# coolbeam/UPFlow_pytorch

Measured on AMD Instinct MI355X. Metric: frame-pairs/sec at 384x1280 bf16, higher is better.
Workload: dtype bf16; 1 GPU; config2: UPFlow_net inference forward (flow fwd+bwd, occlusion masks, SGU on), 384x1280, batch 4 per GPU, random-init weights; global_batch=4, parallelism=replicas x1 (image pairs sharded, no collective), ranks=1, hip_graph=True, capture_fallback=False, steps_in_flight=4, pyramid_convs=HIP (MFMA kernel), pyramid_dtype=fp16

## Files before the change

### upflow_pytorch_amd/csrc/conv_pair.hip

```cpp
#include "conv_kernel.hpp"

namespace upf {
namespace convp {

using conv::f32x16;
using conv::Mma32;
using conv::u32x2;

constexpr int NT = 256;
template <int SA, int SB, int TH> struct Geo {
  static constexpr int MR = SB * (TH - 1) + 3, MC = SB * 31 + 3;
  static constexpr int XO = (SA == 2) ? 1 : 0;
  static constexpr int IR = SA * (MR - 1) + 3, IC = (SA * (MC - 1) + 3 + XO + 1) / 2 * 2;
};

template <typename T, int K0, int C1O, int TH, bool YC8, int SA, int SB>
__global__ __launch_bounds__(NT, 2)
void conv_pair_kernel(const T* __restrict__ x, long long xbs, int xpitch, int Cin, const T* __restrict__ wa, const float* __restrict__ ba, float slope_a,
                      const T* __restrict__ wb, const float* __restrict__ bb, float slope_b, T* __restrict__ y, long long ybs, int ypitch, int C2,
                      int H, int W, int Hm, int Wm, int Ho, int Wo, int tiles_x, int tiles_y) {
  using G = Geo<SA, SB, TH>;
  constexpr int MR = G::MR, MC = G::MC, IR = G::IR, IC = G::IC, XO = G::XO;
  constexpr bool QUAD = (K0 == 0);
  constexpr int KO = QUAD ? 1 : K0;
  constexpr int NSTEP = QUAD ? 3 : ((K0 == 1) ? 5 : 9);
  constexpr int KSB = C1O / 2;
  constexpr int RPWB = TH / 4;
  extern __shared__ __attribute__((aligned(16))) uint4 lds[];
  uint4* in_s = lds;
  uint4* mid_s = lds + (QUAD ? (IR * IC + 1) / 2 : K0 * IR * IC);

  const int bid = xcd_remap(blockIdx.x, gridDim.x);
  const int tx = bid % tiles_x, ty = (bid / tiles_x) % tiles_y, n = bid / (tiles_x * tiles_y);
  const int x0 = tx * 32, y0 = ty * TH;
  const int my0 = SB * y0 - 1, mx0 = SB * x0 - 1;
  const int tid = threadIdx.x, lane = tid & 63, wave = tid >> 6;
  const int px = lane & 31, kg = lane >> 5;

  {
    const uint32_t plane = (uint32_t)(H * xpitch) * 2u;
    __amdgpu_buffer_rsrc_t xr = __builtin_amdgcn_make_buffer_rsrc(const_cast<T*>(x + (size_t)n * xbs), 0, (uint32_t)Cin * plane, 0x00020000);
    const int iy0 = SA * my0 - 1, ix0 = SA * mx0 - 1 - XO;
    for (int item = tid; item < IR * (IC / 2); item += NT) {
      const int ir = item / (IC / 2), pp = item - ir * (IC / 2);
      const int gy = iy0 + ir, gx = ix0 + 2 * pp;
      const bool in = gy >= 0 && gy < H && gx >= 0 && gx < W;
      const uint32_t off = in ? (uint32_t)(gy * xpitch + gx) * 2u : 0x80000000u;
      const uint32_t hm = (gx + 1 < W) ? 0xffffffffu : 0x0000ffffu;
      if constexpr (QUAD) {
        uint32_t ch[4];
#pragma unroll
        for (int c = 0; c < 4; ++c) ch[c] = __builtin_amdgcn_raw_buffer_load_b32(xr, off + (uint32_t)c * plane, 0, 0) & hm;
        uint2 e0, e1;
        e0.x = __builtin_amdgcn_perm(ch[1], ch[0], 0x05040100u); e1.x = __builtin_amdgcn_perm(ch[1], ch[0], 0x07060302u);
        e0.y = __builtin_amdgcn_perm(ch[3], ch[2], 0x05040100u); e1.y = __builtin_amdgcn_perm(ch[3], ch[2], 0x07060302u);
        uint2* q = reinterpret_cast<uint2*>(in_s);
        q[ir * IC + 2 * pp] = e0;
        q[ir * IC + 2 * pp + 1] = e1;
      }
#pragma unroll
      for (int o = 0; o < K0; ++o) {
        uint32_t ch[8];
#pragma unroll
        for (int c = 0; c < 8; ++c)
          ch[c] = __builtin_amdgcn_raw_buffer_load_b32(xr, off + (uint32_t)(8 * o + c) * plane, 0, 0) & hm;
        uint4 e0, e1;
        e0.x = __builtin_amdgcn_perm(ch[1], ch[0], 0x05040100u); e1.x = __builtin_amdgcn_perm(ch[1], ch[0], 0x07060302u);
        e0.y = __builtin_amdgcn_perm(ch[3], ch[2], 0x05040100u); e1.y = __builtin_amdgcn_perm(ch[3], ch[2], 0x07060302u);
        e0.z = __builtin_amdgcn_perm(ch[5], ch[4], 0x05040100u); e1.z = __builtin_amdgcn_perm(ch[5], ch[4], 0x07060302u);
        e0.w = __builtin_amdgcn_perm(ch[7], ch[6], 0x05040100u); e1.w = __builtin_amdgcn_perm(ch[7], ch[6], 0x07060302u);
        in_s[(o * IR + ir) * IC + 2 * pp] = e0;
        in_s[(o * IR + ir) * IC + 2 * pp + 1] = e1;
      }
    }
  }
  uint4 wA[NSTEP];
#pragma unroll
  for (int s = 0; s < NSTEP; ++s) wA[s] = *reinterpret_cast<const uint4*>(wa + ((size_t)s * 64 + lane) * 8);
  constexpr int C1 = 8 * C1O;
  f32x16 biasA;
#pragma unroll
  for (int e = 0; e < 16; ++e) {
    const int c = (e & 3) + 8 * (e >> 2) + 4 * kg;
    biasA[e] = (c < C1) ? ba[c] : 0.f;
  }
  int offA[NSTEP], offA2[NSTEP];
#pragma unroll
  for (int s = 0; s < NSTEP; ++s) {
    int tap, oct;
    if constexpr (QUAD) { tap = 4 * s + 2 * kg; oct = 0; }
    else if constexpr (K0 == 1) { tap = 2 * s + kg; oct = 0; }
    else { tap = s; oct = kg; }
    const int t1 = tap > 8 ? 8 : tap, t2 = tap + 1 > 8 ? 8 : tap + 1;
    offA[s] = (oct * IR + t1 / 3) * IC + t1 % 3 + XO;
    offA2[s] = (t2 / 3) * IC + t2 % 3 + XO;
  }
  __syncthreads();

  {
    constexpr int NPX = MR * MC, NTILE = (NPX + 31) / 32;
    for (int t = wave; t < NTILE; t += 4) {
      const int p = t * 32 + px;
      const bool pv = p < NPX;
      const int pc = pv ? p : NPX - 1;
      const int mr = pc / MC, mc = pc - mr * MC;
      f32x16 acc = biasA;
      if constexpr (QUAD) {
        const uint2* ib = reinterpret_cast<const uint2*>(in_s) + SA * (mr * IC + mc);
#pragma unroll
        for (int s = 0; s < NSTEP; ++s) {
          const uint2 lo = ib[offA[s]], hi = ib[offA2[s]];
          acc = Mma32<T>::mma(wA[s], make_uint4(lo.x, lo.y, hi.x, hi.y), acc);
        }
      } else {
        const uint4* ib = in_s + SA * (mr * IC + mc);
#pragma unroll
        for (int s = 0; s < NSTEP; ++s) acc = Mma32<T>::mma(wA[s], ib[offA[s]], acc);
      }
      const int my = my0 + mr, mx = mx0 + mc;
      const bool inside = my >= 0 && my < Hm && mx >= 0 && mx < Wm;
      if (pv) {
#pragma unroll
        for (int o = 0; o < C1O; ++o) {
          float v[4];
#pragma unroll
          for (int q = 0; q < 4; ++q) { v[q] = acc[4 * o + q]; v[q] = fmaxf(v[q], v[q] * slope_a); }
          u32x2 w2;
          w2.x = inside ? pack2<T>(v[0], v[1]) : 0u;
          w2.y = inside ? pack2<T>(v[2], v[3]) : 0u;
          *reinterpret_cast<u32x2*>(reinterpret_cast<unsigned char*>(&mid_s[(o * MR + mr) * MC + mc]) + kg * 8) = w2;
        }
      }
    }
  }
  uint4 wB[9][KSB];
#pragma unroll
  for (int tap = 0; tap < 9; ++tap)
#pragma unroll
    for (int ks = 0; ks < KSB; ++ks) wB[tap][ks] = *reinterpret_cast<const uint4*>(wb + ((size_t)(tap * KSB + ks) * 64 + lane) * 8);
  f32x16 acc[RPWB];
#pragma unroll
  for (int e = 0; e < 16; ++e) {
    const int c = (e & 3) + 8 * (e >> 2) + 4 * kg;
    const float bv = (c < C2) ? bb[c] : 0.f;
#pragma unroll
    for (int rr = 0; rr < RPWB; ++rr) acc[rr][e] = bv;
  }
  __syncthreads();

#pragma unroll
  for (int tap = 0; tap < 9; ++tap) {
    const int ky = tap / 3, kx = tap - 3 * ky;
#pragma unroll
    for (int ks = 0; ks < KSB; ++ks)
#pragma unroll
      for (int rr = 0; rr < RPWB; ++rr) {
        const int r = wave * RPWB + rr;
        const uint4 b = mid_s[((2 * ks + kg) * MR + SB * r + ky) * MC + SB * px + kx];
        acc[rr] = Mma32<T>::mma(wB[tap][ks], b, acc[rr]);
      }
  }
  if constexpr (!YC8) {
    if (((ypitch & 7) | (int)(ybs & 7) | (int)(reinterpret_cast<uintptr_t>(y) & 15)) == 0) {
      __syncthreads();
      conv::epilogue_wide<T, RPWB>(acc, reinterpret_cast<unsigned char*>(lds) + wave * conv::EPI_WAVE_BYTES, y + (size_t)n * ybs, C2, Ho, Wo,
                                   0, lane, x0, __builtin_amdgcn_readfirstlane(y0 + wave * RPWB), 1, slope_b, ypitch);
      return;
    }
  }
  const int gx = x0 + px;
#pragma unroll
  for (int rr = 0; rr < RPWB; ++rr) {
    const int gy = y0 + wave * RPWB + rr;
    if (gy >= Ho || gx >= Wo) continue;
    if constexpr (YC8) {
      T* yo = y + (size_t)n * ybs;
#pragma unroll
      for (int g = 0; g < 4; ++g) {
        if (8 * g >= C2) continue;
        float v[4];
#pragma unroll
        for (int q = 0; q < 4; ++q) { v[q] = acc[rr][4 * g + q]; v[q] = fmaxf(v[q], v[q] * slope_b); }
        u32x2 o2;
        o2.x = pack2<T>(v[0], v[1]); o2.y = pack2<T>(v[2], v[3]);
        *reinterpret_cast<u32x2*>(yo + (((size_t)g * Ho + gy) * Wo + gx) * 8 + kg * 4) = o2;
      }
    } else {
      typename Elem<T>::store_t* yo = reinterpret_cast<typename Elem<T>::store_t*>(y + (size_t)n * ybs);
#pragma unroll
      for (int e = 0; e < 16; e += 2) {
        const int c = (e & 3) + 8 * (e >> 2) + 4 * kg;
        float v0 = acc[rr][e], v1 = acc[rr][e + 1];
        v0 = fmaxf(v0, v0 * slope_b); v1 = fmaxf(v1, v1 * slope_b);
        const uint32_t p2 = pack2<T>(v0, v1);
        if (c < C2) yo[((size_t)c * Ho + gy) * ypitch + gx] = (typename Elem<T>::store_t)(p2 & 0xffffu);
        if (c + 1 < C2) yo[((size_t)(c + 1) * Ho + gy) * ypitch + gx] = (typename Elem<T>::store_t)(p2 >> 16);
      }
    }
  }
}

struct PairArgs {
  const void* x; long long xbs; int xpitch, Cin; const void* wa; const float* ba; float slope_a; int C1;
  const void* wb; const float* bb; float slope_b; int C2; void* y; long long ybs; int ypitch; int B, H, W; hipStream_t stream;
  int sa, sb;
};

template <typename T, int K0, int C1O, int TH, bool YC8, int SA, int SB>
int launch_pair(const PairArgs& a) {
  using G = Geo<SA, SB, TH>;
  const int Hm = (a.H - 1) / SA + 1, Wm = (a.W - 1) / SA + 1;
  const int Ho = (Hm - 1) / SB + 1, Wo = (Wm - 1) / SB + 1;
  const int tiles_x = cdiv(Wo, 32), tiles_y = cdiv(Ho, TH);
  const size_t ldsb = (size_t)((K0 == 0 ? (G::IR * G::IC + 1) / 2 : K0 * G::IR * G::IC) + C1O * G::MR * G::MC) * 16;
  static LdsOptIn opt;
  auto kern = &conv_pair_kernel<T, K0, C1O, TH, YC8, SA, SB>;
  opt.ensure(reinterpret_cast<const void*>(kern), ldsb);
  hipLaunchKernelGGL(kern, dim3((unsigned)(a.B * tiles_x * tiles_y)), dim3(NT), ldsb, a.stream, (const T*)a.x, a.xbs, a.xpitch, a.Cin,
                     (const T*)a.wa, a.ba, a.slope_a, (const T*)a.wb, a.bb, a.slope_b, (T*)a.y, a.ybs, a.ypitch, a.C2, a.H, a.W, Hm, Wm, Ho, Wo, tiles_x, tiles_y);
  return check_launch("conv_pair_forward");
}

template <typename T, bool YC8>
int dispatch_pair(const PairArgs& a) {
  const int k0 = a.Cin <= 4 ? 0 : (a.Cin <= 8 ? 1 : 2), c1o = a.C1 / 8;
  if (a.sa == 1) {
    if (k0 == 0 && c1o == 2) return launch_pair<T, 0, 2, 8, YC8, 1, 2>(a);
    if (k0 == 0 && c1o == 4) return launch_pair<T, 0, 4, 4, YC8, 1, 2>(a);
    if (k0 == 1 && c1o == 2 && conv::g_pair_th == 4) return launch_pair<T, 1, 2, 4, YC8, 1, 2>(a);
    if (k0 == 1 && c1o == 2) return launch_pair<T, 1, 2, 8, YC8, 1, 2>(a);
    if (k0 == 1 && c1o == 4) return launch_pair<T, 1, 4, 4, YC8, 1, 2>(a);
    if (k0 == 2 && c1o == 2) return launch_pair<T, 2, 2, 8, YC8, 1, 2>(a);
    return launch_pair<T, 2, 4, 4, YC8, 1, 2>(a);
  }
  if constexpr (!YC8) {
    if (k0 == 0 && c1o == 2) return launch_pair<T, 0, 2, 8, false, 2, 1>(a);
    if (k0 == 0 && c1o == 4) return launch_pair<T, 0, 4, 8, false, 2, 1>(a);
    if (k0 == 1 && c1o == 2 && conv::g_pair_th == 4) return launch_pair<T, 1, 2, 4, false, 2, 1>(a);
    if (k0 == 1 && c1o == 2) return launch_pair<T, 1, 2, 8, false, 2, 1>(a);
    if (k0 == 1 && c1o == 4) return launch_pair<T, 1, 4, 8, false, 2, 1>(a);
    if (k0 == 2 && c1o == 2) return launch_pair<T, 2, 2, 8, false, 2, 1>(a);
    return launch_pair<T, 2, 4, 8, false, 2, 1>(a);
  }
  set_error("conv_pair_forward: [stride 2, stride 1] writes NCHW");
  return UPF_EUNSUPPORTED;
}

}
}

extern "C" int upf_conv_pair_forward(const void* x, long long x_batch_stride, int x_row_pitch, int Cin,
                                     const void* wa_packed, const float* bias_a, float slope_a, int C1, int stride_a,
                                     const void* wb_packed, const float* bias_b, float slope_b, int C2, int stride_b,
                                     void* y, long long y_batch_stride, int y_row_pitch, int y_is_c8,
                                     int B, int H, int W, int dtype, void* stream) {
  using namespace upf;
  UPF_REQUIRE(x && wa_packed && bias_a && wb_packed && bias_b && y, UPF_EINVAL, "conv_pair_forward: null pointer");
  UPF_REQUIRE(B > 0 && H > 0 && W > 0, UPF_EINVAL, "conv_pair_forward: bad shape B=%d H=%d W=%d", B, H, W);
  UPF_REQUIRE(dtype == UPF_BF16 || dtype == UPF_F16, UPF_EDTYPE, "conv_pair_forward: bf16 / fp16 only");
  UPF_REQUIRE(Cin >= 1 && Cin <= 16 && (C1 == 16 || C1 == 32) && C2 >= 1 && C2 <= 32, UPF_EUNSUPPORTED,
              "conv_pair_forward: Cin <= 16, C1 = 16 | 32, C2 <= 32 (got %d, %d, %d)", Cin, C1, C2);
  UPF_REQUIRE((stride_a == 1 && stride_b == 2) || (stride_a == 2 && stride_b == 1), UPF_EUNSUPPORTED,
              "conv_pair_forward: strides (1, 2) or (2, 1), got (%d, %d)", stride_a, stride_b);
  if (x_row_pitch == 0) x_row_pitch = W;
  const int Ho = (H - 1) / 2 + 1, Wo = (W - 1) / 2 + 1;
  if (y_row_pitch == 0) y_row_pitch = Wo;
  UPF_REQUIRE(x_row_pitch >= W && x_row_pitch % 2 == 0 && aligned_to(x, 4) && x_batch_stride % 2 == 0, UPF_EUNSUPPORTED,
              "conv_pair_forward: the input rows are read as pixel pairs: an even row pitch (%d) and a 4-byte aligned base", x_row_pitch);
  UPF_REQUIRE(slope_a >= 0.f && slope_a <= 1.f && slope_b >= 0.f && slope_b <= 1.f, UPF_EINVAL, "conv_pair_forward: leaky slopes in [0,1]");
  UPF_REQUIRE(aligned_to(wa_packed, 16) && aligned_to(wb_packed, 16), UPF_EINVAL, "conv_pair_forward: packed weights must be 16-byte aligned");
  UPF_REQUIRE(y_is_c8 ? (aligned_to(y, 16) && y_batch_stride % 8 == 0) : (y_row_pitch >= Wo), UPF_EINVAL, "conv_pair_forward: bad output layout");
  UPF_REQUIRE((long long)Cin * H * x_row_pitch * 2 < (1ll << 31), UPF_EINVAL, "conv_pair_forward: image too large for one buffer descriptor");
  convp::PairArgs a{x, x_batch_stride, x_row_pitch, Cin, wa_packed, bias_a, slope_a == 0.f ? 1.f : slope_a, C1,
                    wb_packed, bias_b, slope_b == 0.f ? 1.f : slope_b, C2, y, y_batch_stride, y_row_pitch, B, H, W, (hipStream_t)stream, stride_a, stride_b};
  if (dtype == UPF_BF16) return y_is_c8 ? convp::dispatch_pair<bf16_t, true>(a) : convp::dispatch_pair<bf16_t, false>(a);
  return y_is_c8 ? convp::dispatch_pair<f16_t, true>(a) : convp::dispatch_pair<f16_t, false>(a);
}
```

Baseline: 1928 frame-pairs/s.

## Software-pipeline LDS loads and MFMAs in fused conv-pair kernel

Restructures the fused two-conv kernel so that global input loads are all issued before the permute/store phase, the first conv's LDS operand fetch is double/triple-buffered ahead of its MFMAs with sched barriers, and the second conv preloads the next kernel row of LDS operands while computing the current one. Adds a spare LDS slot so invalid-pixel stores go to a dummy location instead of branching, and raises the occupancy hint to 3 workgroups for the small quad-input variant when LDS allows. The goal is to hide LDS and global latency behind MFMA work. The cost is higher register pressure, which may cause spills or lower occupancy.

```diff
diff --git a/upflow_pytorch_amd/csrc/conv_pair.hip b/upflow_pytorch_amd/csrc/conv_pair.hip
--- a/upflow_pytorch_amd/csrc/conv_pair.hip
+++ b/upflow_pytorch_amd/csrc/conv_pair.hip
@@ -14,8 +14,16 @@
   static constexpr int IR = SA * (MR - 1) + 3, IC = (SA * (MC - 1) + 3 + XO + 1) / 2 * 2;
 };
 
+template <int K0, int C1O, int TH, int SA, int SB> constexpr int pair_lds_bytes() {
+  using G = Geo<SA, SB, TH>;
+  return ((K0 == 0 ? (G::IR * G::IC + 1) / 2 : K0 * G::IR * G::IC) + C1O * G::MR * G::MC + 1) * 16;
+}
+template <int K0, int C1O, int TH, int SA, int SB> constexpr int pair_min_wg() {
+  return (K0 == 0 && C1O == 2 && 160 * 1024 / pair_lds_bytes<K0, C1O, TH, SA, SB>() >= 3) ? 3 : 2;
+}
+
 template <typename T, int K0, int C1O, int TH, bool YC8, int SA, int SB>
-__global__ __launch_bounds__(NT, 2)
+__global__ __launch_bounds__(NT, (pair_min_wg<K0, C1O, TH, SA, SB>()))
 void conv_pair_kernel(const T* __restrict__ x, long long xbs, int xpitch, int Cin, const T* __restrict__ wa, const float* __restrict__ ba, float slope_a,
                       const T* __restrict__ wb, const float* __restrict__ bb, float slope_b, T* __restrict__ y, long long ybs, int ypitch, int C2,
                       int H, int W, int Hm, int Wm, int Ho, int Wo, int tiles_x, int tiles_y) {
@@ -38,39 +46,53 @@
   const int px = lane & 31, kg = lane >> 5;
 
   {
+    constexpr int NPAIR = IR * (IC / 2), NITEM = (NPAIR + NT - 1) / NT, NPL = QUAD ? 4 : 8 * K0;
     const uint32_t plane = (uint32_t)(H * xpitch) * 2u;
     __amdgpu_buffer_rsrc_t xr = __builtin_amdgcn_make_buffer_rsrc(const_cast<T*>(x + (size_t)n * xbs), 0, (uint32_t)Cin * plane, 0x00020000);
     const int iy0 = SA * my0 - 1, ix0 = SA * mx0 - 1 - XO;
-    for (int item = tid; item < IR * (IC / 2); item += NT) {
-      const int ir = item / (IC / 2), pp = item - ir * (IC / 2);
+    uint32_t ch[NITEM][NPL], hm[NITEM];
+    int dst[NITEM];
+    int ir = tid / (IC / 2), pp = tid - ir * (IC / 2);
+#pragma unroll
+    for (int i = 0; i < NITEM; ++i) {
+      if ((i + 1) * NT > NPAIR) {
+        const bool past = i * NT + tid >= NPAIR;
+        ir = past ? IR - 1 : ir; pp = past ? IC / 2 - 1 : pp;
+      }
       const int gy = iy0 + ir, gx = ix0 + 2 * pp;
-      const bool in = gy >= 0 && gy < H && gx >= 0 && gx < W;
+      const bool in = ((unsigned)gy < (unsigned)H) & ((unsigned)gx < (unsigned)W);
       const uint32_t off = in ? (uint32_t)(gy * xpitch + gx) * 2u : 0x80000000u;
-      const uint32_t hm = (gx + 1 < W) ? 0xffffffffu : 0x0000ffffu;
+      hm[i] = (gx + 1 < W) ? 0xffffffffu : 0x0000ffffu;
+      dst[i] = ir * IC + 2 * pp;
+#pragma unroll
+      for (int c = 0; c < NPL; ++c)
+        ch[i][c] = __builtin_amdgcn_raw_buffer_load_b32(xr, off + (uint32_t)c * plane, 0, 0);
+      ir += NT / (IC / 2); pp += NT % (IC / 2);
+      if (pp >= IC / 2) { pp -= IC / 2; ++ir; }
+    }
+#pragma unroll
+    for (int i = 0; i < NITEM; ++i) {
       if constexpr (QUAD) {
-        uint32_t ch[4];
-#pragma unroll
-        for (int c = 0; c < 4; ++c) ch[c] = __builtin_amdgcn_raw_buffer_load_b32(xr, off + (uint32_t)c * plane, 0, 0) & hm;
+        const uint32_t c0 = ch[i][0] & hm[i], c1 = ch[i][1] & hm[i], c2 = ch[i][2] & hm[i], c3 = ch[i][3] & hm[i];
         uint2 e0, e1;
-        e0.x = __builtin_amdgcn_perm(ch[1], ch[0], 0x05040100u); e1.x = __builtin_amdgcn_perm(ch[1], ch[0], 0x07060302u);
-        e0.y = __builtin_amdgcn_perm(ch[3], ch[2], 0x05040100u); e1.y = __builtin_amdgcn_perm(ch[3], ch[2], 0x07060302u);
+        e0.x = __builtin_amdgcn_perm(c1, c0, 0x05040100u); e1.x = __builtin_amdgcn_perm(c1, c0, 0x07060302u);
+        e0.y = __builtin_amdgcn_perm(c3, c2, 0x05040100u); e1.y = __builtin_amdgcn_perm(c3, c2, 0x07060302u);
         uint2* q = reinterpret_cast<uint2*>(in_s);
-        q[ir * IC + 2 * pp] = e0;
-        q[ir * IC + 2 * pp + 1] = e1;
+        q[dst[i]] = e0;
+        q[dst[i] + 1] = e1;
       }
 #pragma unroll
       for (int o = 0; o < K0; ++o) {
-        uint32_t ch[8];
-#pragma unroll
-        for (int c = 0; c < 8; ++c)
-          ch[c] = __builtin_amdgcn_raw_buffer_load_b32(xr, off + (uint32_t)(8 * o + c) * plane, 0, 0) & hm;
+        uint32_t c[8];
+#pragma unroll
+        for (int j = 0; j < 8; ++j) c[j] = ch[i][8 * o + j] & hm[i];
         uint4 e0, e1;
-        e0.x = __builtin_amdgcn_perm(ch[1], ch[0], 0x05040100u); e1.x = __builtin_amdgcn_perm(ch[1], ch[0], 0x07060302u);
-        e0.y = __builtin_amdgcn_perm(ch[3], ch[2], 0x05040100u); e1.y = __builtin_amdgcn_perm(ch[3], ch[2], 0x07060302u);
-        e0.z = __builtin_amdgcn_perm(ch[5], ch[4], 0x05040100u); e1.z = __builtin_amdgcn_perm(ch[5], ch[4], 0x07060302u);
-        e0.w = __builtin_amdgcn_perm(ch[7], ch[6], 0x05040100u); e1.w = __builtin_amdgcn_perm(ch[7], ch[6], 0x07060302u);
-        in_s[(o * IR + ir) * IC + 2 * pp] = e0;
-        in_s[(o * IR + ir) * IC + 2 * pp + 1] = e1;
+        e0.x = __builtin_amdgcn_perm(c[1], c[0], 0x05040100u); e1.x = __builtin_amdgcn_perm(c[1], c[0], 0x07060302u);
+        e0.y = __builtin_amdgcn_perm(c[3], c[2], 0x05040100u); e1.y = __builtin_amdgcn_perm(c[3], c[2], 0x07060302u);
+        e0.z = __builtin_amdgcn_perm(c[5], c[4], 0x05040100u); e1.z = __builtin_amdgcn_perm(c[5], c[4], 0x07060302u);
+        e0.w = __builtin_amdgcn_perm(c[7], c[6], 0x05040100u); e1.w = __builtin_amdgcn_perm(c[7], c[6], 0x07060302u);
+        in_s[o * IR * IC + dst[i]] = e0;
+        in_s[o * IR * IC + dst[i] + 1] = e1;
       }
     }
   }
@@ -98,39 +120,59 @@
   __syncthreads();
 
   {
-    constexpr int NPX = MR * MC, NTILE = (NPX + 31) / 32;
-    for (int t = wave; t < NTILE; t += 4) {
-      const int p = t * 32 + px;
-      const bool pv = p < NPX;
-      const int pc = pv ? p : NPX - 1;
-      const int mr = pc / MC, mc = pc - mr * MC;
-      f32x16 acc = biasA;
+    constexpr int NPX = MR * MC, NTILE = (NPX + 31) / 32, NIT = (NTILE + 3) / 4;
+    struct Grp { uint4 b[NSTEP]; bool pv, inside; };
+    Grp g[3];
+    f32x16 accA[2];
+    const int p0 = wave * 32 + px;
+    int mr = p0 / MC, mc = p0 - mr * MC;
+    unsigned char* const mid_w = reinterpret_cast<unsigned char*>(&mid_s[p0]) + kg * 8;
+    auto fetch = [&](Grp& q, int k) {
+      const bool last = k == NIT - 1;
+      q.pv = !last || p0 + 128 * k < NPX;
+      const int r = q.pv ? mr : MR - 1, c = q.pv ? mc : MC - 1;
       if constexpr (QUAD) {
-        const uint2* ib = reinterpret_cast<const uint2*>(in_s) + SA * (mr * IC + mc);
+        const uint2* ib = reinterpret_cast<const uint2*>(in_s) + SA * (r * IC + c);
 #pragma unroll
         for (int s = 0; s < NSTEP; ++s) {
           const uint2 lo = ib[offA[s]], hi = ib[offA2[s]];
-          acc = Mma32<T>::mma(wA[s], make_uint4(lo.x, lo.y, hi.x, hi.y), acc);
+          q.b[s] = make_uint4(lo.x, lo.y, hi.x, hi.y);
         }
       } else {
-        const uint4* ib = in_s + SA * (mr * IC + mc);
-#pragma unroll
-        for (int s = 0; s < NSTEP; ++s) acc = Mma32<T>::mma(wA[s], ib[offA[s]], acc);
-      }
-      const int my = my0 + mr, mx = mx0 + mc;
-      const bool inside = my >= 0 && my < Hm && mx >= 0 && mx < Wm;
-      if (pv) {
-#pragma unroll
-        for (int o = 0; o < C1O; ++o) {
-          float v[4];
-#pragma unroll
-          for (int q = 0; q < 4; ++q) { v[q] = acc[4 * o + q]; v[q] = fmaxf(v[q], v[q] * slope_a); }
-          u32x2 w2;
-          w2.x = inside ? pack2<T>(v[0], v[1]) : 0u;
-          w2.y = inside ? pack2<T>(v[2], v[3]) : 0u;
-          *reinterpret_cast<u32x2*>(reinterpret_cast<unsigned char*>(&mid_s[(o * MR + mr) * MC + mc]) + kg * 8) = w2;
-        }
-      }
+        const uint4* ib = in_s + SA * (r * IC + c);
+#pragma unroll
+        for (int s = 0; s < NSTEP; ++s) q.b[s] = ib[offA[s]];
+      }
+      q.inside = ((unsigned)(my0 + r) < (unsigned)Hm) & ((unsigned)(mx0 + c) < (unsigned)Wm);
+      mr += 128 / MC; mc += 128 % MC;
+      if (mc >= MC) { mc -= MC; ++mr; }
+    };
+    auto finish = [&](const Grp& q, const f32x16& a, int k) {
+#pragma unroll
+      for (int o = 0; o < C1O; ++o) {
+        float v[4];
+#pragma unroll
+        for (int e = 0; e < 4; ++e) { v[e] = a[4 * o + e]; v[e] = fmaxf(v[e], v[e] * slope_a); }
+        u32x2 w2;
+        w2.x = q.inside ? pack2<T>(v[0], v[1]) : 0u;
+        w2.y = q.inside ? pack2<T>(v[2], v[3]) : 0u;
+        unsigned char* w = mid_w + (o * MR * MC + 128 * k) * 16;
+        if (k == NIT - 1) w = q.pv ? w : reinterpret_cast<unsigned char*>(&mid_s[C1O * MR * MC]) + kg * 8;
+        *reinterpret_cast<u32x2*>(w) = w2;
+      }
+    };
+    fetch(g[0], 0);
+#pragma unroll
+    for (int k = 0; k <= NIT; ++k) {
+      if (k + 1 < NIT) fetch(g[(k + 1) % 3], k + 1);
+      __builtin_amdgcn_sched_barrier(0);
+      if (k < NIT) {
+        accA[k & 1] = biasA;
+#pragma unroll
+        for (int s = 0; s < NSTEP; ++s) accA[k & 1] = Mma32<T>::mma(wA[s], g[k % 3].b[s], accA[k & 1]);
+      }
+      if (k >= 1) finish(g[(k - 1) % 3], accA[(k - 1) & 1], k - 1);
+      __builtin_amdgcn_sched_barrier(0);
     }
   }
   uint4 wB[9][KSB];
@@ -142,23 +184,38 @@
 #pragma unroll
   for (int e = 0; e < 16; ++e) {
     const int c = (e & 3) + 8 * (e >> 2) + 4 * kg;
-    const float bv = (c < C2) ? bb[c] : 0.f;
+    const float bl = bb[c < C2 ? c : 0], bv = (c < C2) ? bl : 0.f;
 #pragma unroll
     for (int rr = 0; rr < RPWB; ++rr) acc[rr][e] = bv;
   }
   __syncthreads();
 
-#pragma unroll
-  for (int tap = 0; tap < 9; ++tap) {
-    const int ky = tap / 3, kx = tap - 3 * ky;
-#pragma unroll
-    for (int ks = 0; ks < KSB; ++ks)
-#pragma unroll
-      for (int rr = 0; rr < RPWB; ++rr) {
-        const int r = wave * RPWB + rr;
-        const uint4 b = mid_s[((2 * ks + kg) * MR + SB * r + ky) * MC + SB * px + kx];
-        acc[rr] = Mma32<T>::mma(wB[tap][ks], b, acc[rr]);
-      }
+  {
+    constexpr int NB = 3 * KSB * RPWB;
+    uint4 bq[2][NB];
+    auto bload = [&](int ky, uint4 (&b)[NB]) {
+#pragma unroll
+      for (int kx = 0; kx < 3; ++kx)
+#pragma unroll
+        for (int ks = 0; ks < KSB; ++ks)
+#pragma unroll
+          for (int rr = 0; rr < RPWB; ++rr)
+            b[(kx * KSB + ks) * RPWB + rr] = mid_s[((2 * ks + kg) * MR + SB * (wave * RPWB + rr) + ky) * MC + SB * px + kx];
+    };
+    bload(0, bq[0]);
+#pragma unroll
+    for (int ky = 0; ky < 3; ++ky) {
+      if (ky + 1 < 3) bload(ky + 1, bq[(ky + 1) & 1]);
+      __builtin_amdgcn_sched_barrier(0);
+#pragma unroll
+      for (int kx = 0; kx < 3; ++kx)
+#pragma unroll
+        for (int ks = 0; ks < KSB; ++ks)
+#pragma unroll
+          for (int rr = 0; rr < RPWB; ++rr)
+            acc[rr] = Mma32<T>::mma(wB[3 * ky + kx][ks], bq[ky & 1][(kx * KSB + ks) * RPWB + rr], acc[rr]);
+      __builtin_amdgcn_sched_barrier(0);
+    }
   }
   if constexpr (!YC8) {
     if (((ypitch & 7) | (int)(ybs & 7) | (int)(reinterpret_cast<uintptr_t>(y) & 15)) == 0) {
@@ -208,11 +265,10 @@
 
 template <typename T, int K0, int C1O, int TH, bool YC8, int SA, int SB>
 int launch_pair(const PairArgs& a) {
-  using G = Geo<SA, SB, TH>;
   const int Hm = (a.H - 1) / SA + 1, Wm = (a.W - 1) / SA + 1;
   const int Ho = (Hm - 1) / SB + 1, Wo = (Wm - 1) / SB + 1;
   const int tiles_x = cdiv(Wo, 32), tiles_y = cdiv(Ho, TH);
-  const size_t ldsb = (size_t)((K0 == 0 ? (G::IR * G::IC + 1) / 2 : K0 * G::IR * G::IC) + C1O * G::MR * G::MC) * 16;
+  const size_t ldsb = pair_lds_bytes<K0, C1O, TH, SA, SB>();
   static LdsOptIn opt;
   auto kern = &conv_pair_kernel<T, K0, C1O, TH, YC8, SA, SB>;
   opt.ensure(reinterpret_cast<const void*>(kern), ldsb);
```

New measurement: 1938 frame-pairs/s, median of 6. No clear change (+0.5%).

## Restructure conv_pair loads and phase-A loop, tune per-variant launch bounds

Applied to the files above, without the earlier changes.

Replaces the flat per-item input staging loop with a row-per-wave scheme: each lane handles one pixel pair, rows go to waves, and out-of-image rows use a zero-size buffer resource so bounds are not checked per element. Phase A is rewritten around row-aligned 32-pixel steps with precomputed per-step LDS pointers, a separate remainder-column step, an interior fast path that skips border masking, and an inline v_max leaky ReLU. The launch-bounds occupancy hint now varies per template variant instead of a fixed 2. This cuts index arithmetic and divides, but adds code size and register pressure, and the static_asserts limit which geometries compile.

```diff
diff --git a/upflow_pytorch_amd/csrc/conv_pair.hip b/upflow_pytorch_amd/csrc/conv_pair.hip
--- a/upflow_pytorch_amd/csrc/conv_pair.hip
+++ b/upflow_pytorch_amd/csrc/conv_pair.hip
@@ -1,4 +1,5 @@
 #include "conv_kernel.hpp"
+#include <type_traits>
 
 namespace upf {
 namespace convp {
@@ -6,6 +7,13 @@
 using conv::f32x16;
 using conv::Mma32;
 using conv::u32x2;
+
+__device__ __forceinline__ float leaky_max(float v, float slope) {
+  const float sv = v * slope;
+  float r;
+  asm("v_max_f32 %0, %1, %2" : "=v"(r) : "v"(v), "v"(sv));
+  return r;
+}
 
 constexpr int NT = 256;
 template <int SA, int SB, int TH> struct Geo {
@@ -14,8 +22,14 @@
   static constexpr int IR = SA * (MR - 1) + 3, IC = (SA * (MC - 1) + 3 + XO + 1) / 2 * 2;
 };
 
+template <int K0, int C1O, int TH, bool YC8, int SA> constexpr int pair_waves() {
+  if (C1O == 4) return SA == 2 ? 3 : 4;
+  if (TH == 4) return SA == 2 ? 5 : 6;
+  return (YC8 || (SA == 2 && K0 != 0)) ? 5 : 4;
+}
+
 template <typename T, int K0, int C1O, int TH, bool YC8, int SA, int SB>
-__global__ __launch_bounds__(NT, 2)
+__global__ __launch_bounds__(NT, (pair_waves<K0, C1O, TH, YC8, SA>()))
 void conv_pair_kernel(const T* __restrict__ x, long long xbs, int xpitch, int Cin, const T* __restrict__ wa, const float* __restrict__ ba, float slope_a,
                       const T* __restrict__ wb, const float* __restrict__ bb, float slope_b, T* __restrict__ y, long long ybs, int ypitch, int C2,
                       int H, int W, int Hm, int Wm, int Ho, int Wo, int tiles_x, int tiles_y) {
@@ -38,39 +52,51 @@
   const int px = lane & 31, kg = lane >> 5;
 
   {
+    constexpr int NP = IC / 2, NK = (IR + 3) / 4;
+    static_assert(NP <= 64, "conv_pair: a row of pixel pairs per wave instruction");
     const uint32_t plane = (uint32_t)(H * xpitch) * 2u;
     __amdgpu_buffer_rsrc_t xr = __builtin_amdgcn_make_buffer_rsrc(const_cast<T*>(x + (size_t)n * xbs), 0, (uint32_t)Cin * plane, 0x00020000);
+    __amdgpu_buffer_rsrc_t xz = __builtin_amdgcn_make_buffer_rsrc(const_cast<T*>(x + (size_t)n * xbs), 0, 0, 0x00020000);
     const int iy0 = SA * my0 - 1, ix0 = SA * mx0 - 1 - XO;
-    for (int item = tid; item < IR * (IC / 2); item += NT) {
-      const int ir = item / (IC / 2), pp = item - ir * (IC / 2);
-      const int gy = iy0 + ir, gx = ix0 + 2 * pp;
-      const bool in = gy >= 0 && gy < H && gx >= 0 && gx < W;
-      const uint32_t off = in ? (uint32_t)(gy * xpitch + gx) * 2u : 0x80000000u;
-      const uint32_t hm = (gx + 1 < W) ? 0xffffffffu : 0x0000ffffu;
-      if constexpr (QUAD) {
-        uint32_t ch[4];
-#pragma unroll
-        for (int c = 0; c < 4; ++c) ch[c] = __builtin_amdgcn_raw_buffer_load_b32(xr, off + (uint32_t)c * plane, 0, 0) & hm;
-        uint2 e0, e1;
-        e0.x = __builtin_amdgcn_perm(ch[1], ch[0], 0x05040100u); e1.x = __builtin_amdgcn_perm(ch[1], ch[0], 0x07060302u);
-        e0.y = __builtin_amdgcn_perm(ch[3], ch[2], 0x05040100u); e1.y = __builtin_amdgcn_perm(ch[3], ch[2], 0x07060302u);
-        uint2* q = reinterpret_cast<uint2*>(in_s);
-        q[ir * IC + 2 * pp] = e0;
-        q[ir * IC + 2 * pp + 1] = e1;
-      }
-#pragma unroll
-      for (int o = 0; o < K0; ++o) {
-        uint32_t ch[8];
-#pragma unroll
-        for (int c = 0; c < 8; ++c)
-          ch[c] = __builtin_amdgcn_raw_buffer_load_b32(xr, off + (uint32_t)(8 * o + c) * plane, 0, 0) & hm;
-        uint4 e0, e1;
-        e0.x = __builtin_amdgcn_perm(ch[1], ch[0], 0x05040100u); e1.x = __builtin_amdgcn_perm(ch[1], ch[0], 0x07060302u);
-        e0.y = __builtin_amdgcn_perm(ch[3], ch[2], 0x05040100u); e1.y = __builtin_amdgcn_perm(ch[3], ch[2], 0x07060302u);
-        e0.z = __builtin_amdgcn_perm(ch[5], ch[4], 0x05040100u); e1.z = __builtin_amdgcn_perm(ch[5], ch[4], 0x07060302u);
-        e0.w = __builtin_amdgcn_perm(ch[7], ch[6], 0x05040100u); e1.w = __builtin_amdgcn_perm(ch[7], ch[6], 0x07060302u);
-        in_s[(o * IR + ir) * IC + 2 * pp] = e0;
-        in_s[(o * IR + ir) * IC + 2 * pp + 1] = e1;
+    const int wv = __builtin_amdgcn_readfirstlane(wave);
+    const int gx = ix0 + 2 * lane;
+    const uint32_t coff = (gx >= 0 && gx < W) ? (uint32_t)gx * 2u : 0x80000000u;
+    const uint32_t hm = (gx + 1 < W) ? 0xffffffffu : 0x0000ffffu;
+    if (lane < NP) {
+#pragma unroll
+      for (int k = 0; k < NK; ++k) {
+        const int ir = wv + 4 * k;
+        if (4 * k + 3 < IR || ir < IR) {
+          const int gy = iy0 + ir;
+          const bool row_in = gy >= 0 && gy < H;
+          __amdgpu_buffer_rsrc_t r = row_in ? xr : xz;
+          const uint32_t roff = row_in ? (uint32_t)(gy * xpitch) * 2u : 0u;
+          if constexpr (QUAD) {
+            uint32_t ch[4];
+#pragma unroll
+            for (int c = 0; c < 4; ++c) ch[c] = __builtin_amdgcn_raw_buffer_load_b32(r, coff + (uint32_t)c * plane, roff, 0) & hm;
+            uint2 e0, e1;
+            e0.x = __builtin_amdgcn_perm(ch[1], ch[0], 0x05040100u); e1.x = __builtin_amdgcn_perm(ch[1], ch[0], 0x07060302u);
+            e0.y = __builtin_amdgcn_perm(ch[3], ch[2], 0x05040100u); e1.y = __builtin_amdgcn_perm(ch[3], ch[2], 0x07060302u);
+            uint2* q = reinterpret_cast<uint2*>(in_s);
+            q[ir * IC + 2 * lane] = e0;
+            q[ir * IC + 2 * lane + 1] = e1;
+          }
+#pragma unroll
+          for (int o = 0; o < K0; ++o) {
+            uint32_t ch[8];
+#pragma unroll
+            for (int c = 0; c < 8; ++c)
+              ch[c] = __builtin_amdgcn_raw_buffer_load_b32(r, coff + (uint32_t)(8 * o + c) * plane, roff, 0) & hm;
+            uint4 e0, e1;
+            e0.x = __builtin_amdgcn_perm(ch[1], ch[0], 0x05040100u); e1.x = __builtin_amdgcn_perm(ch[1], ch[0], 0x07060302u);
+            e0.y = __builtin_amdgcn_perm(ch[3], ch[2], 0x05040100u); e1.y = __builtin_amdgcn_perm(ch[3], ch[2], 0x07060302u);
+            e0.z = __builtin_amdgcn_perm(ch[5], ch[4], 0x05040100u); e1.z = __builtin_amdgcn_perm(ch[5], ch[4], 0x07060302u);
+            e0.w = __builtin_amdgcn_perm(ch[7], ch[6], 0x05040100u); e1.w = __builtin_amdgcn_perm(ch[7], ch[6], 0x07060302u);
+            in_s[(o * IR + ir) * IC + 2 * lane] = e0;
+            in_s[(o * IR + ir) * IC + 2 * lane + 1] = e1;
+          }
+        }
       }
     }
   }
@@ -84,53 +110,89 @@
     const int c = (e & 3) + 8 * (e >> 2) + 4 * kg;
     biasA[e] = (c < C1) ? ba[c] : 0.f;
   }
-  int offA[NSTEP], offA2[NSTEP];
+  int offA[NSTEP], dA[NSTEP], offA2[NSTEP], dA2[NSTEP];
 #pragma unroll
   for (int s = 0; s < NSTEP; ++s) {
-    int tap, oct;
-    if constexpr (QUAD) { tap = 4 * s + 2 * kg; oct = 0; }
-    else if constexpr (K0 == 1) { tap = 2 * s + kg; oct = 0; }
-    else { tap = s; oct = kg; }
-    const int t1 = tap > 8 ? 8 : tap, t2 = tap + 1 > 8 ? 8 : tap + 1;
-    offA[s] = (oct * IR + t1 / 3) * IC + t1 % 3 + XO;
-    offA2[s] = (t2 / 3) * IC + t2 % 3 + XO;
+    const int t0 = QUAD ? 4 * s : (K0 == 1 ? 2 * s : s), t1 = QUAD ? 4 * s + 2 : (K0 == 1 ? 2 * s + 1 : s);
+    int o[4];
+#pragma unroll
+    for (int j = 0; j < 4; ++j) {
+      const int t = (j & 1 ? t1 : t0) + (j >> 1), tc = t > 8 ? 8 : t;
+      o[j] = (tc / 3) * IC + tc % 3 + XO;
+    }
+    offA[s] = o[0]; dA[s] = o[1] - o[0] + (K0 == 2 ? IR * IC : 0);
+    offA2[s] = o[2]; dA2[s] = o[3] - o[2];
   }
   __syncthreads();
 
   {
-    constexpr int NPX = MR * MC, NTILE = (NPX + 31) / 32;
-    for (int t = wave; t < NTILE; t += 4) {
-      const int p = t * 32 + px;
-      const bool pv = p < NPX;
-      const int pc = pv ? p : NPX - 1;
-      const int mr = pc / MC, mc = pc - mr * MC;
+    constexpr int G = MC / 32, REM = MC % 32, RS = 4 / G;
+    constexpr int NFULL = MR * G, NI = (NFULL + 3) / 4;
+    static_assert((G == 1 || G == 2) && (REM == 1 || REM == 2) && REM * MR <= 32, "conv_pair: the row-aligned steps of phase A");
+    using E = typename std::conditional<QUAD, uint2, uint4>::type;
+    const E* in_e = reinterpret_cast<const E*>(in_s);
+    const int wv = __builtin_amdgcn_readfirstlane(wave);
+    const bool interior = my0 >= 0 && my0 + MR <= Hm && mx0 >= 0 && mx0 + MC <= Wm;
+    auto put = [&](const f32x16& acc, unsigned char* md, auto border, bool keep) {
+#pragma unroll
+      for (int o = 0; o < C1O; ++o) {
+        float v[4];
+#pragma unroll
+        for (int q = 0; q < 4; ++q) v[q] = leaky_max(acc[4 * o + q], slope_a);
+        u32x2 w2;
+        w2.x = pack2<T>(v[0], v[1]);
+        w2.y = pack2<T>(v[2], v[3]);
+        if constexpr (decltype(border)::value) { w2.x = keep ? w2.x : 0u; w2.y = keep ? w2.y : 0u; }
+        *reinterpret_cast<u32x2*>(md + o * (MR * MC * 16)) = w2;
+      }
+    };
+    auto step = [&](const E* const (&ia)[NSTEP], const E* const (&ia2)[NSTEP], int eo, unsigned char* md, bool valid, bool keep) {
       f32x16 acc = biasA;
-      if constexpr (QUAD) {
-        const uint2* ib = reinterpret_cast<const uint2*>(in_s) + SA * (mr * IC + mc);
-#pragma unroll
-        for (int s = 0; s < NSTEP; ++s) {
-          const uint2 lo = ib[offA[s]], hi = ib[offA2[s]];
+#pragma unroll
+      for (int s = 0; s < NSTEP; ++s) {
+        if constexpr (QUAD) {
+          const uint2 lo = ia[s][eo + offA[s]], hi = ia2[s][eo + offA2[s]];
           acc = Mma32<T>::mma(wA[s], make_uint4(lo.x, lo.y, hi.x, hi.y), acc);
+        } else {
+          acc = Mma32<T>::mma(wA[s], ia[s][eo + offA[s]], acc);
         }
-      } else {
-        const uint4* ib = in_s + SA * (mr * IC + mc);
-#pragma unroll
-        for (int s = 0; s < NSTEP; ++s) acc = Mma32<T>::mma(wA[s], ib[offA[s]], acc);
-      }
-      const int my = my0 + mr, mx = mx0 + mc;
-      const bool inside = my >= 0 && my < Hm && mx >= 0 && mx < Wm;
-      if (pv) {
-#pragma unroll
-        for (int o = 0; o < C1O; ++o) {
-          float v[4];
-#pragma unroll
-          for (int q = 0; q < 4; ++q) { v[q] = acc[4 * o + q]; v[q] = fmaxf(v[q], v[q] * slope_a); }
-          u32x2 w2;
-          w2.x = inside ? pack2<T>(v[0], v[1]) : 0u;
-          w2.y = inside ? pack2<T>(v[2], v[3]) : 0u;
-          *reinterpret_cast<u32x2*>(reinterpret_cast<unsigned char*>(&mid_s[(o * MR + mr) * MC + mc]) + kg * 8) = w2;
+      }
+      if (valid) {
+        if (interior) put(acc, md, std::false_type(), true);
+        else put(acc, md, std::true_type(), keep);
+      }
+    };
+    {
+      const int mr0 = wv / G, mc = 32 * (wv % G) + px;
+      const E* ia[NSTEP];
+      const E* ia2[NSTEP];
+#pragma unroll
+      for (int s = 0; s < NSTEP; ++s) {
+        ia[s] = in_e + SA * (mr0 * IC + mc) + kg * dA[s];
+        ia2[s] = in_e + SA * (mr0 * IC + mc) + kg * dA2[s];
+      }
+      unsigned char* md = reinterpret_cast<unsigned char*>(&mid_s[mr0 * MC + mc]) + kg * 8;
+      const bool col_in = (unsigned)(mx0 + mc) < (unsigned)Wm;
+#pragma unroll
+      for (int i = 0; i < NI; ++i) {
+        if (4 * i + 3 < NFULL || wv + 4 * i < NFULL) {
+          const bool row_in = (unsigned)(my0 + mr0 + RS * i) < (unsigned)Hm;
+          step(ia, ia2, i * (RS * SA * IC), md + i * (RS * MC * 16), true, row_in && col_in);
         }
       }
+    }
+    if (wv == NFULL % 4) {
+      const bool pv = px < REM * MR;
+      const int mr = pv ? px / REM : MR - 1, mc = 32 * G + px % REM;
+      const E* ia[NSTEP];
+      const E* ia2[NSTEP];
+#pragma unroll
+      for (int s = 0; s < NSTEP; ++s) {
+        ia[s] = in_e + SA * (mr * IC + mc) + kg * dA[s];
+        ia2[s] = in_e + SA * (mr * IC + mc) + kg * dA2[s];
+      }
+      unsigned char* md = reinterpret_cast<unsigned char*>(&mid_s[mr * MC + mc]) + kg * 8;
+      step(ia, ia2, 0, md, pv, (unsigned)(my0 + mr) < (unsigned)Hm && (unsigned)(mx0 + mc) < (unsigned)Wm);
     }
   }
   uint4 wB[9][KSB];
```

Result: no change. 1960 frame-pairs/s before, 1974 frame-pairs/s after, median of 6 (+0.7%).
